# adityaX1412/Experiment-YOLO

Hardware: AMD Instinct MI355X
Metric: images/sec (train) DEAL-YOLO-N 640x640 bs=64/GPU (higher is better)
Workload: dtype f16; 1 GPU; DEAL-YOLO-N (yolov8n-ASF-P2P2.yaml) train step 640x640, per-GPU batch 64, fwd+TAL/WIOU+NWD/DFL/BCE loss+bwd+SGD+EMA, BASELINE.json configs[1]; loss_mode=wiou+nwd, settle_steps=18, capture_retries=0, global_batch=64, parallelism=dp1, hipgraph=True

## Files before the change

### experiment-yolo_amd/csrc/common.h

```cpp
#pragma once
#include <type_traits>
#include <hip/hip_runtime.h>
#include <stdint.h>

typedef _Float16 f16;
typedef _Float16 half8 __attribute__((ext_vector_type(8)));
typedef _Float16 half4 __attribute__((ext_vector_type(4)));
typedef _Float16 half2_ __attribute__((ext_vector_type(2)));
typedef float f32x4 __attribute__((ext_vector_type(4)));
typedef float f32x2 __attribute__((ext_vector_type(2)));

#define DY_OK 0
#define DY_ERR_ARG (-1)
#define DY_ERR_LAUNCH (-2)
#define DY_ERR_ALIGN (-3)
#define DY_ERR_CAPACITY (-4)

#define LDS_AS __attribute__((address_space(3)))

static __device__ __forceinline__ float wave_sum(float v) {
#pragma unroll
  for (int o = 32; o > 0; o >>= 1) v += __shfl_xor(v, o, 64);
  return v;
}
static __device__ __forceinline__ float wave_max(float v) {
#pragma unroll
  for (int o = 32; o > 0; o >>= 1) v = fmaxf(v, __shfl_xor(v, o, 64));
  return v;
}
template <int CTRL>
static __device__ __forceinline__ float dpp_read(float x) {
  return __builtin_bit_cast(float, __builtin_amdgcn_update_dpp(0, __builtin_bit_cast(int, x), CTRL, 0xF, 0xF, true));
}
#define DY_DPP_QUAD_1032 0xB1
#define DY_DPP_QUAD_2301 0x4E
#define DY_DPP_HALF_MIRROR 0x141
// ... 62 lines not shown
    const f32x2 den = (f32x2){__builtin_amdgcn_exp2f(t[0]), __builtin_amdgcn_exp2f(t[1])} + (f32x2){1.f, 1.f};
    const f32x2 s = {__builtin_amdgcn_rcpf(den[0]), __builtin_amdgcn_rcpf(den[1])};
    const f32x2 q = __builtin_elementwise_fma(-s, s, s);
    return __builtin_elementwise_fma(z, q, s);
  }
  if (ACT == DY_ACT_LEAKY) return (f32x2){z[0] > 0.f ? 1.f : 0.1f, z[1] > 0.f ? 1.f : 0.1f};
  return (f32x2){1.f, 1.f};
}
template <int ACT>
static __device__ __forceinline__ float act_grad_t(float z) {
  return act_grad2<ACT>((f32x2){z, z})[0];
}
template <int ACT>
static __device__ __forceinline__ half8 bn_bwd_apply8(const half8& dv, const half8& xv, const float* sc, const float* sh,
                                                      const float* kb, const float* kc) {
  half8 out;
#pragma unroll
  for (int j = 0; j < 8; j += 2) {
    const f32x2 x = {(float)xv[j], (float)xv[j + 1]}, d = {(float)dv[j], (float)dv[j + 1]};
    const f32x2 s2 = {sc[j], sc[j + 1]}, h2 = {sh[j], sh[j + 1]}, b2 = {kb[j], kb[j + 1]}, c2 = {kc[j], kc[j + 1]};
    const f32x2 ad = act_grad2<ACT>(__builtin_elementwise_fma(x, s2, h2));
    const f32x2 o = __builtin_elementwise_fma(s2 * ad, d, -__builtin_elementwise_fma(b2, x, c2));
    const half2_ oh = __builtin_convertvector(o, half2_);
    out[j] = oh[0];
    out[j + 1] = oh[1];
  }
  return out;
}

#define DY_NUM_CUS 256

static inline int cdiv(int a, int b) { return (a + b - 1) / b; }

#define DY_CHECK_LAUNCH()                                  \
  do {                                                     \
    hipError_t e__ = hipGetLastError();                    \
    if (e__ != hipSuccess) return DY_ERR_LAUNCH;           \
  } while (0)
```

### experiment-yolo_amd/csrc/head_rows.hip

```cpp
#include <hip/hip_runtime.h>

#include <cstdlib>

#include "common.h"
#include "dealyolo_hip.h"

template <typename T>
struct Levels {
  int nl;
  T lv[4];
};
struct RowsArgs {
  const f16* x;
  const f16* dy;
  const int* flag;
  const float* w;
  f16* dx;
  float* slabs;
  double* bias_acc;
  int ldx, lddy, lddx, A, a0, hw, B, dx_acc;
  const float* xcoef;
  int nblk, dgx;
};

__global__ __launch_bounds__(256) void rows_wgrad_kernel(Levels<RowsArgs> L) {
  const RowsArgs& a = L.lv[blockIdx.y];
  if ((int)blockIdx.x >= a.nblk) return;
  __shared__ int s_list[256];
  __shared__ int s_cnt[4];
  __shared__ __attribute__((aligned(16))) f16 s_x[16 * 64], s_dy[16 * 64];
  const int tid = threadIdx.x, wave = tid >> 6, lane = tid & 63;
  const int co = tid >> 2, ci0 = (tid & 3) * 16;
  const long npix = (long)a.B * a.hw;
  const long chunk = (npix + a.nblk - 1) / a.nblk;
  const long lo = (long)blockIdx.x * chunk, hi = lo + chunk < npix ? lo + chunk : npix;
  float acc[16];
#pragma unroll
  for (int k = 0; k < 16; ++k) acc[k] = 0.f;
  float bs = 0.f;
  constexpr int FB = 8;
  int fl[FB];
  for (long p0 = lo, trip = 0; p0 < hi; p0 += 256, ++trip) {
    if ((trip & (FB - 1)) == 0) {
#pragma unroll
      for (int k = 0; k < FB; ++k) {
        const long pk = p0 + (long)k * 256 + tid;
        fl[k] = -1;
        if (pk < hi) {
          const int b = (int)(pk / a.hw), r = (int)(pk - (long)b * a.hw);
          fl[k] = a.flag[(size_t)b * a.A + a.a0 + r];
        }
      }
    }
    int mine = -1;
#pragma unroll
    for (int k = 0; k < FB; ++k)
      if ((trip & (FB - 1)) == k) mine = fl[k];
    const bool fg = mine >= 0;
    const unsigned long long m = __ballot(fg);
    if (lane == 0) s_cnt[wave] = __popcll(m);
    __syncthreads();
    int base = 0, total = 0;
#pragma unroll
    for (int w = 0; w < 4; ++w) {
      if (w < wave) base += s_cnt[w];
      total += s_cnt[w];
    }
    if (fg) s_list[base + __popcll(m & ((1ull << lane) - 1ull))] = tid;
    __syncthreads();
    for (int i0 = 0; i0 < total; i0 += 16) {
      const int nb = total - i0 < 16 ? total - i0 : 16;
      {
        const int i = tid >> 4, g = tid & 15;
        if (i < nb) {
          const long q = p0 + s_list[i0 + i];
          if (g < 8) {
            half8 xv = *reinterpret_cast<const half8*>(a.x + q * a.ldx + g * 8);
            if (a.xcoef) xv = bn_silu_apply8(xv, a.xcoef + g * 8, a.xcoef + 64 + g * 8);
            *reinterpret_cast<half8*>(s_x + i * 64 + g * 8) = xv;
          } else {
            *reinterpret_cast<uint4*>(s_dy + i * 64 + (g - 8) * 8) = *reinterpret_cast<const uint4*>(a.dy + q * a.lddy + (g - 8) * 8);
          }
        }
      }
      __syncthreads();
      for (int i = 0; i < nb; ++i) {
        const float g = (float)s_dy[i * 64 + co];
#pragma unroll
        for (int k = 0; k < 16; ++k) acc[k] += g * (float)s_x[i * 64 + ci0 + k];
        if ((tid & 3) == 0) bs += g;
      }
      __syncthreads();
    }
  }
  float* slab = a.slabs + (size_t)blockIdx.x * 64 * 64 + co * 64 + ci0;
#pragma unroll
  for (int k = 0; k < 16; k += 4) *reinterpret_cast<float4*>(slab + k) = make_float4(acc[k], acc[k + 1], acc[k + 2], acc[k + 3]);
  if ((tid & 3) == 0 && bs != 0.f) unsafeAtomicAdd(a.bias_acc + (size_t)(blockIdx.x % DY_BN_COPIES) * 64 + co, (double)bs);
}

__global__ __launch_bounds__(256) void rows_dgrad_kernel(Levels<RowsArgs> L) {
  const RowsArgs& a = L.lv[blockIdx.z];
  if (!a.dx || (int)blockIdx.x >= a.dgx || (int)blockIdx.y >= a.B) return;
  __shared__ float s_w[64 * 65];
  for (int i = threadIdx.x; i < 64 * 64; i += 256) s_w[(i >> 6) * 65 + (i & 63)] = (float)(f16)a.w[i];
  __syncthreads();
  const int b = blockIdx.y, part = threadIdx.x & 7, ci0 = part * 8;
  const int* const fl = a.flag + (size_t)b * a.A + a.a0;
  for (int r = (int)(blockIdx.x * 32 + (threadIdx.x >> 3)); r < a.hw; r += a.dgx * 32) {
    const long p = (long)b * a.hw + r;
    f16* const dst = a.dx + p * a.lddx + ci0;
    if (fl[r] < 0) {
      if (!a.dx_acc) *reinterpret_cast<uint4*>(dst) = make_uint4(0, 0, 0, 0);
      continue;
    }
    float s[8];
#pragma unroll
    for (int k = 0; k < 8; ++k) s[k] = 0.f;
    const f16* const g = a.dy + p * a.lddy;
    for (int c8 = 0; c8 < 64; c8 += 8) {
      const half8 gv = *reinterpret_cast<const half8*>(g + c8);
#pragma unroll
      for (int j = 0; j < 8; ++j) {
        const float gg = (float)gv[j];
#pragma unroll
        for (int k = 0; k < 8; ++k) s[k] += gg * s_w[(c8 + j) * 65 + ci0 + k];
      }
    }
    half8 o;
    if (a.dx_acc) {
      const half8 old = *reinterpret_cast<const half8*>(dst);
#pragma unroll
      for (int k = 0; k < 8; ++k) o[k] = (f16)((float)old[k] + s[k]);
    } else {
#pragma unroll
      for (int k = 0; k < 8; ++k) o[k] = (f16)s[k];
    }
    *reinterpret_cast<half8*>(dst) = o;
  }
}

static __device__ __forceinline__ float exp_nonpos(float x) {
  const float t = x * 1.44269502f;
  float r = __builtin_fmaf(x, 1.44269502f, -t);
  r = __builtin_fmaf(x, 1.92596299e-8f, r);
  const float e = __builtin_amdgcn_exp2f(t);
  return __builtin_fmaf(e, r * 0.693147182f, e);
}
static __device__ __forceinline__ f32x2 exp_nonpos2(f32x2 x) {
  const f32x2 l2e = {1.44269502f, 1.44269502f}, l2e_lo = {1.92596299e-8f, 1.92596299e-8f}, ln2 = {0.693147182f, 0.693147182f};
  const f32x2 t = x * l2e;
  f32x2 r = __builtin_elementwise_fma(x, l2e, -t);
  r = __builtin_elementwise_fma(x, l2e_lo, r);
  const f32x2 e = {__builtin_amdgcn_exp2f(t[0]), __builtin_amdgcn_exp2f(t[1])};
  return __builtin_elementwise_fma(e, r * ln2, e);
}
struct BoxDecArgs {
  const f16* x;
  const float* w;
  const float* bias;
  float* pred_box;
  int ldx, A, a0, hw, W, B;
  const float* xcoef;
  int nblk;
};
template <bool LIBM>
__global__ __launch_bounds__(256) void head_box_decode_kernel(Levels<BoxDecArgs> L) {
  const BoxDecArgs& a = L.lv[blockIdx.y];
  if ((int)blockIdx.x >= a.nblk) return;
  auto ex = [](float x) { return LIBM ? expf(x) : exp_nonpos(x); };
  constexpr int PITCH = 160;
// ... 120 lines not shown
    const int rc = box_decode_fill(L.lv[l], x[l], ldx[l], x_coef ? x_coef[l] : nullptr, weight[l], bias[l], pred_box, A, a0[l], n, h[l], w[l], cin, cout);
    if (rc != DY_OK) return rc;
  }
  return box_decode_launch(L, stream);
}

extern "C" int dy_conv1x1_rows_supported(int cin, int cout) { return cin == 64 && cout == 64; }
extern "C" int dy_conv1x1_rows_slabs(int n, int h, int w) {
  const long ns = (long)n * h * w / 2048;
  return ns < 64 ? 64 : (ns > 1024 ? 1024 : (int)ns);
}
static int rows_fill(RowsArgs& a, const void* x, int ldx, const float* x_coef, const void* dy, int lddy, const int* assigned, int A, int a0,
                     const float* weight, void* dx, int lddx, int dx_accumulate, float* slabs, double* bias_acc, int n, int h, int w, int cin,
                     int cout) {
  if (!dy_conv1x1_rows_supported(cin, cout) || !x || !dy || !assigned || !weight || !slabs || !bias_acc || n < 1 || h < 1 || w < 1 ||
      a0 < 0 || a0 + h * w > A)
    return DY_ERR_ARG;
  if ((ldx & 7) || (lddy & 7) || (dx && (lddx & 7)) || ((uintptr_t)x & 15) || ((uintptr_t)dy & 15) || ((uintptr_t)dx & 15) ||
      ((uintptr_t)slabs & 15))
    return DY_ERR_ALIGN;
  int gx = (h * w + 1023) / 1024;
  if (gx > 16) gx = 16;
  a = RowsArgs{(const f16*)x, (const f16*)dy, assigned, weight, (f16*)dx, slabs, bias_acc, ldx, lddy, lddx, A, a0, h * w, n, dx_accumulate, x_coef,
               dy_conv1x1_rows_slabs(n, h, w), gx};
  return DY_OK;
}
static int rows_launch(const Levels<RowsArgs>& L, hipStream_t stream) {
  int gw = 1, gd = 0, nb = 1;
  for (int l = 0; l < L.nl; ++l) {
    gw = L.lv[l].nblk > gw ? L.lv[l].nblk : gw;
    if (L.lv[l].dx) gd = L.lv[l].dgx > gd ? L.lv[l].dgx : gd;
    nb = L.lv[l].B > nb ? L.lv[l].B : nb;
  }
  hipLaunchKernelGGL(rows_wgrad_kernel, dim3(gw, L.nl), dim3(256), 0, stream, L);
  if (gd) hipLaunchKernelGGL(rows_dgrad_kernel, dim3(gd, nb, L.nl), dim3(256), 0, stream, L);
  DY_CHECK_LAUNCH();
  return DY_OK;
}
extern "C" int dy_conv1x1_rows_backward(const void* x, int ldx, const float* x_coef, const void* dy, int lddy, const int* assigned, int A, int a0,
                                        const float* weight, void* dx, int lddx, int dx_accumulate, float* slabs, double* bias_acc,
                                        int n, int h, int w, int cin, int cout, hipStream_t stream) {
  Levels<RowsArgs> L{};
  L.nl = 1;
  const int rc = rows_fill(L.lv[0], x, ldx, x_coef, dy, lddy, assigned, A, a0, weight, dx, lddx, dx_accumulate, slabs, bias_acc, n, h, w, cin, cout);
  return rc != DY_OK ? rc : rows_launch(L, stream);
}
extern "C" int dy_conv1x1_rows_backward_levels(int nl, const void* const* x, const int* ldx, const float* const* x_coef, const void* const* dy,
                                               const int* lddy, const int* assigned, int A, const int* a0, const float* const* weight,
                                               void* const* dx, const int* lddx, const int* dx_accumulate, float* const* slabs,
                                               double* const* bias_acc, int n, const int* h, const int* w, int cin, int cout,
                                               hipStream_t stream) {
  if (nl < 1 || nl > 4) return DY_ERR_ARG;
  Levels<RowsArgs> L{};
  L.nl = nl;
  for (int l = 0; l < nl; ++l) {
    const int rc = rows_fill(L.lv[l], x[l], ldx[l], x_coef ? x_coef[l] : nullptr, dy[l], lddy[l], assigned, A, a0[l], weight[l], dx[l], lddx[l],
                             dx_accumulate[l], slabs[l], bias_acc[l], n, h[l], w[l], cin, cout);
    if (rc != DY_OK) return rc;
  }
  return rows_launch(L, stream);
}

struct ClsArgs {
  const f16* x;
  const float* xcoef;
  const float* w;
  const float* bias;
  float* y;
// ... 213 lines not shown
```

### experiment-yolo_amd/csrc/loss.hip

```cpp
#include "common.h"
#include "dealyolo_hip.h"

#define REG_MAX 16
#define TOPK 10
#define TAL_EPS 1e-9f
#define IOU_EPS 1e-7f

struct Level {
  const float* box;
  const float* cls;
  f16* dbox;
  f16* dcls;
  int H, W, a0;
  float stride;
  const f16* xin = nullptr;
  int ldin = 0;
  const float* w = nullptr;
  const float* bias = nullptr;
  const float* incoef = nullptr;
};
struct BoxMode {
  int family, ltype, fm, modifier;
  float inner_ratio, focaler_d, focaler_u, shape_scale, piou_lambda;
  float mpd_hw_num;
// ... 317 lines not shown
      const Dual scw = sx * 0.5f + IOU_EPS, sch = sy * 0.5f + IOU_EPS;
      const Dual sigma = t_sqrt(dsq(scw) + dsq(sch));
      const Dual s1 = dabs(scw) / sigma, s2 = dabs(sch) / sigma;
      const Dual sa = dsel(s1.v > 0.70710678118654752f, s2, s1);
      const Dual gamma = dcos(dasin(sa) * 2.f - (float)(M_PI / 2)) - 2.f;
      const Dual dc = (2.f - t_exp(gamma * dsq(scw / cw))) - t_exp(gamma * dsq(sch / ch));
      const Dual ow = dabs(w1 - w2) / dmaximum(w1, dconst(w2)), oh = dabs(h1 - h2) / dmaximum(h1, dconst(h2));
      const Dual sc = dpow4(1.f - t_exp(-ow)) + dpow4(1.f - t_exp(-oh));
      return (I - 0.5f * (dc + sc)) + IOU_EPS;
    }
    case DY_BOX_SHAPEIOU: {
      const float pws = powf(w2, m.shape_scale), phs = powf(h2, m.shape_scale);
      const float ww = 2.f * pws / (pws + phs), hh = 2.f * phs / (pws + phs);
      const Dual dist = (hh * (dsq(sx) / 4.f) + ww * (dsq(sy) / 4.f)) / c2;
      const Dual ow = (hh * dabs(w1 - w2)) / dmaximum(w1, dconst(w2)), oh = (ww * dabs(h1 - h2)) / dmaximum(h1, dconst(h2));
      const Dual sc = dpow4(1.f - t_exp(-ow)) + dpow4(1.f - t_exp(-oh));
      return (I - dist) - 0.5f * sc;
    }
    case DY_BOX_PIOU:
    case DY_BOX_PIOU2: {
      const Dual dw1 = dabs(dminimum(x2, x1) - fminf(t[2], t[0])), dw2 = dabs(dmaximum(x2, x1) - fmaxf(t[2], t[0]));
      const Dual dh1 = dabs(dminimum(y2, y1) - fminf(t[3], t[1])), dh2 = dabs(dmaximum(y2, y1) - fmaxf(t[3], t[1]));
      const Dual P = ((dw1 + dw2) / fabsf(w2) + (dh1 + dh2) / fabsf(h2)) / 4.f;
      const Dual pv1 = ((1.f - I) - t_exp(-dsq(P))) + 1.f;
      if (m.ltype == DY_BOX_PIOU) return 1.f - pv1;
      const Dual x = t_exp(-P) * m.piou_lambda;
      return 1.f - ((3.f * x) * t_exp(-dsq(x))) * pv1;
    }
    default:
      return I - rho2 / c2;
  }
}

__global__ void pack_targets_kernel(LossCtx c, const float* bidx, const float* cls, const float* boxes, int n,
                                    const int* n_dev, float img_w, float img_h) {
  if (n_dev) n = *n_dev;
  for (int i = blockIdx.x * blockDim.x + threadIdx.x; i < c.B * c.nmax; i += gridDim.x * blockDim.x) {
    c.gt_valid[i] = 0;
    c.gt_cls[i] = 0;
    c.pos_align[i] = 0u;
    c.pos_ov[i] = 0u;
    for (int k = 0; k < 4; ++k) c.gt_box[i * 4 + k] = 0.f;
  }
  if (threadIdx.x == 0) c.scal[9] = 0.f;
  __shared__ short sb[8192];
  const int ncache = n < 8192 ? n : 8192;
  for (int i = threadIdx.x; i < ncache; i += blockDim.x) sb[i] = (short)(int)bidx[i];
  __syncthreads();
  for (int i = threadIdx.x; i < n; i += blockDim.x) {
    const int b = (int)bidx[i];
    if (b < 0 || b >= c.B) continue;
    int slot = 0;
    for (int j = 0; j < i; ++j) slot += ((j < ncache ? (int)sb[j] : (int)bidx[j]) == b);
    if (slot >= c.nmax) {
      c.scal[9] = 1.f;
      c.scal[10] = 1.f;
      continue;
    }
    const float x = boxes[i * 4 + 0] * img_w, y = boxes[i * 4 + 1] * img_h;
    const float w = boxes[i * 4 + 2] * img_w, h = boxes[i * 4 + 3] * img_h;
    const float dw = w / 2, dh = h / 2;
    float* g = c.gt_box + ((size_t)b * c.nmax + slot) * 4;
    g[0] = x - dw; g[1] = y - dh; g[2] = x + dw; g[3] = y + dh;
    c.gt_cls[b * c.nmax + slot] = (int)cls[i];
    c.gt_valid[b * c.nmax + slot] = (g[0] + g[1] + g[2] + g[3]) > 0.f ? 1 : 0;
  }
}

static __device__ __forceinline__ float softmax16_expect(float logit, int bin, float& prob) {
  float m = logit;
  m = fmaxf(m, __shfl_xor(m, 1, 64));
  m = fmaxf(m, __shfl_xor(m, 2, 64));
  m = fmaxf(m, __shfl_xor(m, 4, 64));
  m = fmaxf(m, __shfl_xor(m, 8, 64));
  const float e = expf(logit - m);
  const float s = quad16_sum(e);
  prob = e / s;
  return quad16_sum(prob * (float)bin);
}

__global__ __launch_bounds__(256) void decode_kernel(LossCtx c) {
  const int sub = threadIdx.x & 15, side = sub >> 2, quarter = sub & 3;
  const int b = blockIdx.y;
  float invw[4];
#pragma unroll
  for (int k = 0; k < 4; ++k) invw[k] = k < c.nl ? 1.0f / (float)c.lv[k].W : 0.f;
  for (int a = (int)((blockIdx.x * 256 + threadIdx.x) >> 4); a < c.A; a += (int)((gridDim.x * 256) >> 4)) {
    int l = 0;
#pragma unroll
    for (int k = 1; k < 4; ++k)
      if (k < c.nl && a >= c.lv[k].a0) l = k;
    const Level& L = c.lv[l];
    const int r = a - L.a0;
    const int iy = (int)(((float)r + 0.5f) * invw[l]), ix = r - iy * L.W;
    const float4 v = *reinterpret_cast<const float4*>(L.box + ((size_t)b * (L.H * L.W) + r) * 64 + sub * 4);
    float m = fmaxf(fmaxf(v.x, v.y), fmaxf(v.z, v.w));
    m = fmaxf(m, __shfl_xor(m, 1, 64));
    m = fmaxf(m, __shfl_xor(m, 2, 64));
    const float e0 = expf(v.x - m), e1 = expf(v.y - m), e2 = expf(v.z - m), e3 = expf(v.w - m);
    float den = (e0 + e1) + (e2 + e3);
    const float k0 = (float)(quarter * 4);
    float num = e0 * k0 + e1 * (k0 + 1.f) + e2 * (k0 + 2.f) + e3 * (k0 + 3.f);
    den += __shfl_xor(den, 1, 64);
    num += __shfl_xor(num, 1, 64);
    den += __shfl_xor(den, 2, 64);
    num += __shfl_xor(num, 2, 64);
    const float e = num / den;
    const float anc = (side & 1) ? (iy + 0.5f) : (ix + 0.5f);
    if (quarter == 0) c.pred_box[((size_t)b * c.A + a) * 4 + side] = side < 2 ? anc - e : anc + e;
  }
}

#define TAL_CAP 2048
__global__ __launch_bounds__(256) void tal_topk_kernel(LossCtx c) {
  const int bj = blockIdx.x, b = bj / c.nmax, tid = threadIdx.x;
  __shared__ float s_m[TAL_CAP + TOPK];
  __shared__ int s_a[TAL_CAP + TOPK];
  __shared__ float r_m[256];
  __shared__ int r_i[256];
  __shared__ int s_keep;
  int* out = c.topk_idx + (size_t)bj * TOPK;
  if (tid < TOPK) out[tid] = -1;
  if (!c.gt_valid[bj]) return;
  const float* g = c.gt_box + (size_t)bj * 4;
  const float gx1 = g[0], gy1 = g[1], gx2 = g[2], gy2 = g[3];
  const int label = c.gt_cls[bj];
  int x0[4], y0[4], nx[4], ny[4], cum[5];
  cum[0] = 0;
  for (int l = 0; l < 4; ++l) {
    x0[l] = y0[l] = nx[l] = ny[l] = 0;
    if (l < c.nl) {
      const float s = c.lv[l].stride;
      int xa = (int)floorf(gx1 / s - 0.5f) - 1, xb = (int)ceilf(gx2 / s - 0.5f) + 1;
      int ya = (int)floorf(gy1 / s - 0.5f) - 1, yb = (int)ceilf(gy2 / s - 0.5f) + 1;
      xa = xa < 0 ? 0 : xa; ya = ya < 0 ? 0 : ya;
      xb = xb > c.lv[l].W - 1 ? c.lv[l].W - 1 : xb;
      yb = yb > c.lv[l].H - 1 ? c.lv[l].H - 1 : yb;
      x0[l] = xa; y0[l] = ya;
      nx[l] = xb >= xa ? xb - xa + 1 : 0;
      ny[l] = yb >= ya ? yb - ya + 1 : 0;
    }
    cum[l + 1] = cum[l] + nx[l] * ny[l];
  }
  const int ncand = cum[4];
  if (tid == 0) s_keep = 0;
  __syncthreads();
// ... 8 lines not shown
        if (k >= cum[q]) l = q;
      const int r = k - cum[l];
      const int iy = y0[l] + r / nx[l], ix = x0[l] + r % nx[l];
      const float s = c.lv[l].stride;
      const float ax = (ix + 0.5f) * s, ay = (iy + 0.5f) * s;
      const float dmin_ = fminf(fminf(ax - gx1, ay - gy1), fminf(gx2 - ax, gy2 - ay));
      float metric = 0.f;
      const int a = c.lv[l].a0 + iy * c.lv[l].W + ix;
      if (dmin_ > TAL_EPS) {
        const float* pb = c.pred_box + ((size_t)b * c.A + a) * 4;
        const float pp[4] = {pb[0] * s, pb[1] * s, pb[2] * s, pb[3] * s};
        float ov = ciou_gt_pred(g, pp);
        ov = ov > 0.f ? ov : 0.f;
        const float logit = c.lv[l].cls[(((size_t)b * c.lv[l].H + iy) * c.lv[l].W + ix) * c.ncp + label];
        const float sc = c.prob_scores ? logit : 1.f / (1.f + expf(-logit));
        const float o3 = ov * ov * ov;
        metric = sqrtf(sc) * (o3 * o3);
      }
      s_m[keep + t] = metric;
      s_a[keep + t] = a;
    }
    __syncthreads();
    const int n = keep + chunk;
    for (int round = 0; round < TOPK; ++round) {
      float bm = 0.f;
      int bi = -1;
      for (int t = round + tid; t < n; t += 256) {
        const float m = s_m[t];
        if (m > bm || (m == bm && m > 0.f && bi >= 0 && s_a[t] < s_a[bi])) {
          bm = m;
          bi = t;
        }
      }
      r_m[tid] = bm;
      r_i[tid] = bi;
      __syncthreads();
      for (int o = 128; o > 0; o >>= 1) {
        if (tid < o) {
          const float m2 = r_m[tid + o];
          const int i2 = r_i[tid + o];
          const float m1 = r_m[tid];
          const int i1 = r_i[tid];
          if (i2 >= 0 && (i1 < 0 || m2 > m1 || (m2 == m1 && s_a[i2] < s_a[i1]))) {
            r_m[tid] = m2;
            r_i[tid] = i2;
          }
        }
        __syncthreads();
      }
      const int win = r_i[0];
      if (win < 0) {
        if (tid == 0) s_keep = round;
        __syncthreads();
        break;
      }
      if (tid == 0) {
        const float tm = s_m[round];
        const int ta = s_a[round];
        s_m[round] = s_m[win];
        s_a[round] = s_a[win];
        s_m[win] = tm;
        s_a[win] = ta;
        s_keep = round + 1;
      }
      __syncthreads();
    }
    __syncthreads();
  }
  const int keep = s_keep;
  if (tid < keep) out[tid] = s_a[tid];
}

__global__ void tal_scatter_kernel(LossCtx c) {
  const int total = c.B * c.nmax * TOPK;
  for (int i = blockIdx.x * blockDim.x + threadIdx.x; i < total; i += gridDim.x * blockDim.x) {
    const int a = c.topk_idx[i];
    if (a < 0) continue;
    const int bj = i / TOPK, b = bj / c.nmax, j = bj - b * c.nmax;
    atomicAdd(&c.cnt[(size_t)b * c.A + a], 1);
    c.owner[(size_t)b * c.A + a] = j;
  }
}

// ... 85 lines not shown
  __syncthreads();
  for (int o = 128; o > 0; o >>= 1) {
    if (threadIdx.x < o)
      for (int k = 0; k < 3; ++k) red[k][threadIdx.x] += red[k][threadIdx.x + o];
    __syncthreads();
  }
  if (threadIdx.x < 3) c.partials[blockIdx.x * 3 + threadIdx.x] = red[threadIdx.x][0];
}

__global__ __launch_bounds__(256) void loss_scalars_kernel(LossCtx c, int nparts) {
  __shared__ double red[3][256];
  double s[3] = {0, 0, 0};
  for (int i = threadIdx.x; i < nparts; i += 256)
    for (int k = 0; k < 3; ++k) s[k] += c.partials[i * 3 + k];
  for (int k = 0; k < 3; ++k) red[k][threadIdx.x] = s[k];
  __syncthreads();
  for (int o = 128; o > 0; o >>= 1) {
    if (threadIdx.x < o)
      for (int k = 0; k < 3; ++k) red[k][threadIdx.x] += red[k][threadIdx.x + o];
    __syncthreads();
  }
  if (threadIdx.x == 0) {
    const float tss = (float)red[0][0];
    c.scal[0] = tss;
    c.scal[1] = tss > 1.f ? tss : 1.f;
    c.scal[2] = (float)red[1][0];
    c.scal[3] = (float)red[2][0];
    if (c.use_wiou && red[2][0] > 0.0)
      c.scal[4] = c.scal[4] * (1.f - 1e-2f) + 1e-2f * (float)(red[1][0] / red[2][0]);
    c.scal[5] = c.scal[6] = c.scal[7] = c.scal[8] = 0.f;
  }
}

__global__ __launch_bounds__(256) void cls_loss_kernel(LossCtx c, int level) {
  const Level& L = c.lv[level];
  const int hw = L.H * L.W;
  const int npix = c.B * hw;
  const float k = c.hyp_cls * (float)c.B / c.scal[1] * c.gscale[0];
  float acc = 0.f;
  for (int pix = blockIdx.x * 256 + threadIdx.x; pix < npix; pix += gridDim.x * 256) {
    const int b = pix / hw;
    const long ba = (long)b * c.A + L.a0 + (pix - b * hw);
    const int j = c.asg_gt[ba];
    const int tc = j >= 0 ? c.gt_cls[b * c.nmax + j] : -1;
    const float ts = j >= 0 ? c.tscore[ba] : 0.f;
    const float* xp = L.cls + (size_t)pix * c.ncp;
    for (int c0 = 0; c0 < c.ncp; c0 += 8) {
      const float4 v0 = *reinterpret_cast<const float4*>(xp + c0), v1 = *reinterpret_cast<const float4*>(xp + c0 + 4);
      const float xs[8] = {v0.x, v0.y, v0.z, v0.w, v1.x, v1.y, v1.z, v1.w};
      half8 g8;
#pragma unroll
      for (int q = 0; q < 8; ++q) {
        const int cc = c0 + q;
        float g = 0.f;
        if (cc < c.nc) {
          const float x = xs[q], t = cc == tc ? ts : 0.f;
          const float e = __expf(-fabsf(x));
          acc += fmaxf(x, 0.f) - x * t + __logf(1.f + e);
          const float r = __builtin_amdgcn_rcpf(1.f + e);
          g = ((x >= 0.f ? r : e * r) - t) * k;
        }
        g8[q] = (f16)g;
      }
      if (L.dcls) *reinterpret_cast<half8*>(L.dcls + (size_t)pix * c.ncp + c0) = g8;
    }
  }
  __shared__ float red[256];
  red[threadIdx.x] = acc;
  __syncthreads();
  for (int o = 128; o > 0; o >>= 1) {
    if (threadIdx.x < o) red[threadIdx.x] += red[threadIdx.x + o];
    __syncthreads();
  }
  if (threadIdx.x == 0) c.partials[blockIdx.x] = red[0];
}

template <bool EXT>
__global__ __launch_bounds__(256) void box_loss_kernel(LossCtx c) {
  const int lane = threadIdx.x & 63, side = lane >> 4, bin = lane & 15;
  const long wave = ((long)blockIdx.x * 256 + threadIdx.x) >> 6, nw = ((long)gridDim.x * 256) >> 6;
  const long total = (long)c.B * c.A;
  const float tss = c.scal[1], gs = c.gscale[0], Bf = (float)c.B;
  float l_box = 0.f, l_dfl = 0.f;
  for (long base = wave * 64; base < total; base += nw * 64) {
   const int jl = (base + lane < total) ? c.asg_gt[base + lane] : -1;
   unsigned long long fgm = __ballot(jl >= 0);
   while (fgm) {
    const int bit = __ffsll((long long)fgm) - 1;
    fgm &= fgm - 1;
    const long ba = base + bit;
    const int j = __shfl(jl, bit, 64);
    const int b = (int)(ba / c.A), a = (int)(ba - (long)b * c.A);
    int l, iy, ix;
    anchor_of(c, a, l, iy, ix);
    const Level& L = c.lv[l];
    const size_t off = (((size_t)b * L.H + iy) * L.W + ix) * 64 + lane;
    float logit;
    if (L.box) {
      logit = L.box[off];
    } else {
      const float xraw = (float)L.xin[(((size_t)b * L.H + iy) * L.W + ix) * L.ldin + lane];
      float yv = xraw;
      if (L.incoef) {
        const float z = __builtin_fmaf(xraw, L.incoef[lane], L.incoef[64 + lane]);
        const f32x2 a2 = act_fwd2_fast<DY_ACT_SILU>((f32x2){z, z});
        yv = (float)(f16)a2[0];
      }
// ... 157 lines not shown
  return DY_OK;
}

extern "C" int dy_tal_assign(const float* const* scores, const int* H, const int* W, const float* stride, int nl, int B, int nc,
                             int ncp, int n, const float* pd_boxes_grid, const int* gt_labels, const float* gt_bboxes,
                             const int* mask_gt, int* asg_gt, float* tscore, void* workspace, hipStream_t stream) {
  if (nl < 1 || nl > 4 || n < 1 || (ncp & 7) || nc > ncp || !workspace || !asg_gt || !tscore) return DY_ERR_ARG;
  LossCtx c{};
  c.nl = nl; c.B = B; c.nc = nc; c.ncp = ncp; c.nmax = n; c.prob_scores = 1;
  int a0 = 0;
  for (int l = 0; l < nl; ++l) {
    c.lv[l] = Level{nullptr, scores[l], nullptr, nullptr, H[l], W[l], a0, stride[l]};
    a0 += H[l] * W[l];
  }
  c.A = a0;
  char* p = (char*)workspace;
  auto take = [&](size_t b) { char* r = p; p += (b + 255) / 256 * 256; return r; };
  const size_t BA = (size_t)B * c.A, BN = (size_t)B * n;
  take(BN * 16); take(BN * 4); take(BN * 4); take(BA * 16);
  c.gt_box = const_cast<float*>(gt_bboxes); c.gt_cls = const_cast<int*>(gt_labels); c.gt_valid = const_cast<int*>(mask_gt);
  c.pred_box = const_cast<float*>(pd_boxes_grid);
  c.cnt = (int*)take(BA * 4); c.owner = (int*)take(BA * 4);
  take(BA * 4);
  c.asg_gt = asg_gt;
  c.asg_metric = (float*)take(BA * 4); c.asg_ov = (float*)take(BA * 4);
  take(BA * 4);
  c.tscore = tscore;
  c.topk_idx = (int*)take(BN * TOPK * 4); c.pos_align = (unsigned*)take(BN * 4); c.pos_ov = (unsigned*)take(BN * 4);
  take(16 * 4);
  c.partials = (float*)take(3 * 4096 * 4);
  if (hipMemsetAsync(c.cnt, 0, BA * 4, stream) != hipSuccess || hipMemsetAsync(c.pos_align, 0, BN * 4, stream) != hipSuccess ||
      hipMemsetAsync(c.pos_ov, 0, BN * 4, stream) != hipSuccess)
    return DY_ERR_LAUNCH;
  hipLaunchKernelGGL(tal_topk_kernel, dim3((int)BN), dim3(256), 0, stream, c);
  hipLaunchKernelGGL(tal_scatter_kernel, dim3(cdiv((int)BN * TOPK, 256)), dim3(256), 0, stream, c);
  const int gridE = (int)((BA + 255) / 256 < 2048 ? (BA + 255) / 256 : 2048);
  hipLaunchKernelGGL(tal_resolve_kernel, dim3(gridE), dim3(256), 0, stream, c);
  hipLaunchKernelGGL(tal_scores_kernel, dim3(gridE), dim3(256), 0, stream, c);
  DY_CHECK_LAUNCH();
  return DY_OK;
}

extern "C" int dy_loss_args_bytes(void) { return (int)sizeof(DyLossArgs); }
extern "C" int dy_detection_loss(const DyLossArgs* d, hipStream_t stream) {
  if (d->nl < 1 || d->nl > 4 || d->nmax < 1 || (d->ncp & 7) || d->nc > d->ncp) return DY_ERR_ARG;
  LossCtx c{};
  c.nl = d->nl; c.B = d->B; c.nc = d->nc; c.ncp = d->ncp; c.nmax = d->nmax;
  int a0 = 0;
  for (int l = 0; l < d->nl; ++l) {
    c.lv[l] = Level{d->box[l], d->cls[l], (f16*)d->dbox[l], (f16*)d->dcls[l], d->H[l], d->W[l], a0, d->stride[l]};
    if (d->box_from_input) {
      if (!d->box_in[l] || !d->box_w[l] || !d->box_b[l] || (d->box_in_ld[l] & 7)) return DY_ERR_ARG;
      c.lv[l].box = nullptr;
      c.lv[l].xin = (const f16*)d->box_in[l]; c.lv[l].ldin = d->box_in_ld[l]; c.lv[l].w = d->box_w[l]; c.lv[l].bias = d->box_b[l];
      c.lv[l].incoef = d->box_in_coef[l];
    }
    a0 += d->H[l] * d->W[l];
  }
  c.A = a0;
  char* p = (char*)d->workspace;
  auto take = [&](size_t b) { char* r = p; p += (b + 255) / 256 * 256; return r; };
  const size_t BA = (size_t)c.B * c.A, BN = (size_t)c.B * c.nmax;
  c.gt_box = (float*)take(BN * 16); c.gt_cls = (int*)take(BN * 4); c.gt_valid = (int*)take(BN * 4);
  c.pred_box = (float*)take(BA * 16); c.cnt = (int*)take(BA * 4); c.owner = (int*)take(BA * 4);
  c.asg_gt = (int*)take(BA * 4); c.asg_metric = (float*)take(BA * 4); c.asg_ov = (float*)take(BA * 4);
  c.tscore = (float*)take(BA * 4);
  c.topk_idx = (int*)take(BN * TOPK * 4); c.pos_align = (unsigned*)take(BN * 4); c.pos_ov = (unsigned*)take(BN * 4);
  float* scal_ws = (float*)take(16 * 4);
  (void)scal_ws;
  c.scal = d->scalars;
  float* partA = (float*)take(3 * 4096 * 4);
  float* partB = (float*)take(2 * 4096 * 4);
  float* partC = (float*)take(4 * 4096 * 4);
  c.hyp_box = d->hyp_box; c.hyp_cls = d->hyp_cls; c.hyp_dfl = d->hyp_dfl;
  c.use_wiou = d->use_wiou; c.use_nwd = d->use_nwd; c.iou_ratio = d->iou_ratio; c.gscale = d->gscale;
  if (d->box_family != DY_BOX_FAMILY_LEGACY) {
    const int fam = d->box_family, lt = d->box_ltype, mod = d->box_modifier;
    if (fam != DY_BOX_FAMILY_WISE && fam != DY_BOX_FAMILY_BBOX) return DY_ERR_ARG;
    if (lt < DY_BOX_IOU || lt > DY_BOX_MPDIOU || (fam == DY_BOX_FAMILY_BBOX && lt == DY_BOX_WIOU)) return DY_ERR_ARG;
    if (mod < DY_BOX_MOD_PLAIN || mod > DY_BOX_MOD_FOCALER) return DY_ERR_ARG;
    if (fam == DY_BOX_FAMILY_WISE && (d->box_fm < DY_BOX_FM_V1 || d->box_fm > DY_BOX_FM_V3)) return DY_ERR_ARG;
    if (mod == DY_BOX_MOD_FOCALER && !(d->focaler_u != d->focaler_d)) return DY_ERR_ARG;
    c.bm = BoxMode{fam, lt, d->box_fm, mod, d->inner_ratio, d->focaler_d, d->focaler_u, d->shape_scale, d->piou_lambda,
                   d->img_h * d->img_h + d->img_w * d->img_w};
    c.use_wiou = fam == DY_BOX_FAMILY_WISE;
  }

  hipLaunchKernelGGL(pack_targets_kernel, dim3(1), dim3(1024), 0, stream, c, d->t_batch_idx, d->t_cls, d->t_boxes,
                     d->n_targets, d->n_targets_dev, d->img_w, d->img_h);
  if (hipMemsetAsync(c.cnt, 0, BA * 4, stream) != hipSuccess) return DY_ERR_LAUNCH;
  const int gridA = (int)((BA * 64 + 255) / 256 < 2048 ? (BA * 64 + 255) / 256 : 2048);
  if (!d->box_from_input) {
    const long nb = ((long)c.A * 16 + 255) / 256;
    hipLaunchKernelGGL(decode_kernel, dim3((int)(nb < 256 ? nb : 256), c.B), dim3(256), 0, stream, c);
  }
  hipLaunchKernelGGL(tal_topk_kernel, dim3((int)BN), dim3(256), 0, stream, c);
  hipLaunchKernelGGL(tal_scatter_kernel, dim3(cdiv((int)BN * TOPK, 256)), dim3(256), 0, stream, c);
  const int gridE = (int)((BA + 255) / 256 < 2048 ? (BA + 255) / 256 : 2048);
  hipLaunchKernelGGL(tal_resolve_kernel, dim3(gridE), dim3(256), 0, stream, c);
  c.partials = partA;
  hipLaunchKernelGGL(tal_scores_kernel, dim3(gridE), dim3(256), 0, stream, c);
  hipLaunchKernelGGL(loss_scalars_kernel, dim3(1), dim3(256), 0, stream, c, gridE);
  int n_cls = 0;
  for (int l = 0; l < c.nl; ++l) {
    const long tot = (long)c.B * c.lv[l].H * c.lv[l].W;
    int g = (int)((tot + 255) / 256 < 2048 ? (tot + 255) / 256 : 2048);
    c.partials = partC + n_cls;
    hipLaunchKernelGGL(cls_loss_kernel, dim3(g), dim3(256), 0, stream, c, l);
    n_cls += g;
  }
  c.partials = partB;
  for (int l = 0; l < c.nl; ++l)
    if (c.lv[l].dbox && !d->dbox_rows_only && hipMemsetAsync(c.lv[l].dbox, 0, (size_t)c.B * c.lv[l].H * c.lv[l].W * 64 * 2, stream) != hipSuccess)
      return DY_ERR_LAUNCH;
  if (c.bm.family != DY_BOX_FAMILY_LEGACY)
    hipLaunchKernelGGL(box_loss_kernel<true>, dim3(gridA), dim3(256), 0, stream, c);
  else
    hipLaunchKernelGGL(box_loss_kernel<false>, dim3(gridA), dim3(256), 0, stream, c);
  hipLaunchKernelGGL(loss_final_kernel, dim3(1), dim3(256), 0, stream, c, partB, gridA, partC, n_cls);
  DY_CHECK_LAUNCH();
  return DY_OK;
}
```

Measured before the change: 6240 images/s.

## Fuse head row kernels, merge per-level cls loss, speed up target packing and topk

Merges the rows wgrad and dgrad kernels into one launch that splits the grid between the two bodies, and merges the per-level cls_loss launches into a single kernel indexed by level start offsets. Replaces the serial O(n^2) slot counting in target packing with a ballot-based ranking using a shared per-image counter, and replaces the block-wide shared-memory argmax tree in TAL top-k with a wave shuffle reduction plus a 4-entry cross-wave step. The aim is fewer kernel launches and less serialization in small loss kernels. The old paths stay available through the DY_HEAD_V1 environment variable. The new pack kernel zero-fills buffers itself, and the loss path that uses it does not memset pos_align or pos_ov first.

Measured after the change: 6263 images/s (median of 6 runs). No clear change (+0.4%).

```diff
diff --git a/experiment-yolo_amd/csrc/common.h b/experiment-yolo_amd/csrc/common.h
--- a/experiment-yolo_amd/csrc/common.h
+++ b/experiment-yolo_amd/csrc/common.h
@@ -2,6 +2,7 @@
 #include <type_traits>
 #include <hip/hip_runtime.h>
 #include <stdint.h>
+#include <stdlib.h>
 
 typedef _Float16 f16;
 typedef _Float16 half8 __attribute__((ext_vector_type(8)));
@@ -130,6 +131,11 @@
 
 static inline int cdiv(int a, int b) { return (a + b - 1) / b; }
 
+static inline bool dy_head_v1() {
+  const char* e = getenv("DY_HEAD_V1");
+  return e && e[0] == '1' && !e[1];
+}
+
 #define DY_CHECK_LAUNCH()                                  \
   do {                                                     \
     hipError_t e__ = hipGetLastError();                    \
diff --git a/experiment-yolo_amd/csrc/head_rows.hip b/experiment-yolo_amd/csrc/head_rows.hip
--- a/experiment-yolo_amd/csrc/head_rows.hip
+++ b/experiment-yolo_amd/csrc/head_rows.hip
@@ -23,17 +23,18 @@
   int nblk, dgx;
 };
 
-__global__ __launch_bounds__(256) void rows_wgrad_kernel(Levels<RowsArgs> L) {
-  const RowsArgs& a = L.lv[blockIdx.y];
-  if ((int)blockIdx.x >= a.nblk) return;
-  __shared__ int s_list[256];
-  __shared__ int s_cnt[4];
-  __shared__ __attribute__((aligned(16))) f16 s_x[16 * 64], s_dy[16 * 64];
+constexpr int ROWS_LDS = 64 * 65 * 4;
+static __device__ __forceinline__ void rows_wgrad_body(const RowsArgs& a, const int bx, char* smem) {
+  if (bx >= a.nblk) return;
+  int* const s_list = reinterpret_cast<int*>(smem);
+  int* const s_cnt = s_list + 256;
+  f16* const s_x = reinterpret_cast<f16*>(smem + 1040);
+  f16* const s_dy = s_x + 16 * 64;
   const int tid = threadIdx.x, wave = tid >> 6, lane = tid & 63;
   const int co = tid >> 2, ci0 = (tid & 3) * 16;
   const long npix = (long)a.B * a.hw;
   const long chunk = (npix + a.nblk - 1) / a.nblk;
-  const long lo = (long)blockIdx.x * chunk, hi = lo + chunk < npix ? lo + chunk : npix;
+  const long lo = (long)bx * chunk, hi = lo + chunk < npix ? lo + chunk : npix;
   float acc[16];
 #pragma unroll
   for (int k = 0; k < 16; ++k) acc[k] = 0.f;
@@ -93,21 +94,24 @@
       __syncthreads();
     }
   }
-  float* slab = a.slabs + (size_t)blockIdx.x * 64 * 64 + co * 64 + ci0;
+  float* slab = a.slabs + (size_t)bx * 64 * 64 + co * 64 + ci0;
 #pragma unroll
   for (int k = 0; k < 16; k += 4) *reinterpret_cast<float4*>(slab + k) = make_float4(acc[k], acc[k + 1], acc[k + 2], acc[k + 3]);
-  if ((tid & 3) == 0 && bs != 0.f) unsafeAtomicAdd(a.bias_acc + (size_t)(blockIdx.x % DY_BN_COPIES) * 64 + co, (double)bs);
-}
-
-__global__ __launch_bounds__(256) void rows_dgrad_kernel(Levels<RowsArgs> L) {
-  const RowsArgs& a = L.lv[blockIdx.z];
-  if (!a.dx || (int)blockIdx.x >= a.dgx || (int)blockIdx.y >= a.B) return;
-  __shared__ float s_w[64 * 65];
+  if ((tid & 3) == 0 && bs != 0.f) unsafeAtomicAdd(a.bias_acc + (size_t)(bx % DY_BN_COPIES) * 64 + co, (double)bs);
+}
+__global__ __launch_bounds__(256) void rows_wgrad_kernel(Levels<RowsArgs> L) {
+  __shared__ __attribute__((aligned(16))) char smem[1040 + 2 * 16 * 64 * 2];
+  rows_wgrad_body(L.lv[blockIdx.y], (int)blockIdx.x, smem);
+}
+
+static __device__ __forceinline__ void rows_dgrad_body(const RowsArgs& a, const int bx, const int b, char* smem) {
+  if (!a.dx || bx >= a.dgx || b >= a.B) return;
+  float* const s_w = reinterpret_cast<float*>(smem);
   for (int i = threadIdx.x; i < 64 * 64; i += 256) s_w[(i >> 6) * 65 + (i & 63)] = (float)(f16)a.w[i];
   __syncthreads();
-  const int b = blockIdx.y, part = threadIdx.x & 7, ci0 = part * 8;
+  const int part = threadIdx.x & 7, ci0 = part * 8;
   const int* const fl = a.flag + (size_t)b * a.A + a.a0;
-  for (int r = (int)(blockIdx.x * 32 + (threadIdx.x >> 3)); r < a.hw; r += a.dgx * 32) {
+  for (int r = (int)(bx * 32 + (threadIdx.x >> 3)); r < a.hw; r += a.dgx * 32) {
     const long p = (long)b * a.hw + r;
     f16* const dst = a.dx + p * a.lddx + ci0;
     if (fl[r] < 0) {
@@ -137,6 +141,21 @@
       for (int k = 0; k < 8; ++k) o[k] = (f16)s[k];
     }
     *reinterpret_cast<half8*>(dst) = o;
+  }
+}
+__global__ __launch_bounds__(256, 3) void rows_dgrad_kernel(Levels<RowsArgs> L) {
+  __shared__ __attribute__((aligned(16))) char smem[ROWS_LDS];
+  rows_dgrad_body(L.lv[blockIdx.z], (int)blockIdx.x, (int)blockIdx.y, smem);
+}
+__global__ __launch_bounds__(256, 3) void rows_bwd_kernel(Levels<RowsArgs> L, const int gw, const int gd) {
+  __shared__ __attribute__((aligned(16))) char smem[ROWS_LDS];
+  const RowsArgs& a = L.lv[blockIdx.y];
+  const int bx = (int)blockIdx.x;
+  if (bx < gw) {
+    rows_wgrad_body(a, bx, smem);
+  } else {
+    const int i = bx - gw;
+    rows_dgrad_body(a, i % gd, i / gd, smem);
   }
 }
 
@@ -323,8 +342,12 @@
     if (L.lv[l].dx) gd = L.lv[l].dgx > gd ? L.lv[l].dgx : gd;
     nb = L.lv[l].B > nb ? L.lv[l].B : nb;
   }
-  hipLaunchKernelGGL(rows_wgrad_kernel, dim3(gw, L.nl), dim3(256), 0, stream, L);
-  if (gd) hipLaunchKernelGGL(rows_dgrad_kernel, dim3(gd, nb, L.nl), dim3(256), 0, stream, L);
+  if (gd && !dy_head_v1()) {
+    hipLaunchKernelGGL(rows_bwd_kernel, dim3(gw + gd * nb, L.nl), dim3(256), 0, stream, L, gw, gd);
+  } else {
+    hipLaunchKernelGGL(rows_wgrad_kernel, dim3(gw, L.nl), dim3(256), 0, stream, L);
+    if (gd) hipLaunchKernelGGL(rows_dgrad_kernel, dim3(gd, nb, L.nl), dim3(256), 0, stream, L);
+  }
   DY_CHECK_LAUNCH();
   return DY_OK;
 }
diff --git a/experiment-yolo_amd/csrc/loss.hip b/experiment-yolo_amd/csrc/loss.hip
--- a/experiment-yolo_amd/csrc/loss.hip
+++ b/experiment-yolo_amd/csrc/loss.hip
@@ -373,6 +373,21 @@
   }
 }
 
+static __device__ __forceinline__ void pack_fill(const LossCtx& c, const int i, const int b, const int slot, const float* cls,
+                                                 const float* boxes, const float img_w, const float img_h) {
+  if (slot >= c.nmax) {
+    c.scal[9] = 1.f;
+    c.scal[10] = 1.f;
+    return;
+  }
+  const float x = boxes[i * 4 + 0] * img_w, y = boxes[i * 4 + 1] * img_h;
+  const float w = boxes[i * 4 + 2] * img_w, h = boxes[i * 4 + 3] * img_h;
+  const float dw = w / 2, dh = h / 2;
+  float* g = c.gt_box + ((size_t)b * c.nmax + slot) * 4;
+  g[0] = x - dw; g[1] = y - dh; g[2] = x + dw; g[3] = y + dh;
+  c.gt_cls[b * c.nmax + slot] = (int)cls[i];
+  c.gt_valid[b * c.nmax + slot] = (g[0] + g[1] + g[2] + g[3]) > 0.f ? 1 : 0;
+}
 __global__ void pack_targets_kernel(LossCtx c, const float* bidx, const float* cls, const float* boxes, int n,
                                     const int* n_dev, float img_w, float img_h) {
   if (n_dev) n = *n_dev;
@@ -393,18 +408,55 @@
     if (b < 0 || b >= c.B) continue;
     int slot = 0;
     for (int j = 0; j < i; ++j) slot += ((j < ncache ? (int)sb[j] : (int)bidx[j]) == b);
-    if (slot >= c.nmax) {
-      c.scal[9] = 1.f;
-      c.scal[10] = 1.f;
-      continue;
-    }
-    const float x = boxes[i * 4 + 0] * img_w, y = boxes[i * 4 + 1] * img_h;
-    const float w = boxes[i * 4 + 2] * img_w, h = boxes[i * 4 + 3] * img_h;
-    const float dw = w / 2, dh = h / 2;
-    float* g = c.gt_box + ((size_t)b * c.nmax + slot) * 4;
-    g[0] = x - dw; g[1] = y - dh; g[2] = x + dw; g[3] = y + dh;
-    c.gt_cls[b * c.nmax + slot] = (int)cls[i];
-    c.gt_valid[b * c.nmax + slot] = (g[0] + g[1] + g[2] + g[3]) > 0.f ? 1 : 0;
+    pack_fill(c, i, b, slot, cls, boxes, img_w, img_h);
+  }
+}
+
+#define PACK_MAXB 4096
+__global__ __launch_bounds__(1024) void pack_targets_fast_kernel(LossCtx c, const float* bidx, const float* cls, const float* boxes, int n,
+                                                                 const int* n_dev, float img_w, float img_h) {
+  if (n_dev) n = *n_dev;
+  const int tid = threadIdx.x, wave = tid >> 6, lane = tid & 63;
+  for (int i = tid; i < c.B * c.nmax; i += 1024) {
+    c.gt_valid[i] = 0;
+    c.gt_cls[i] = 0;
+    c.pos_align[i] = 0u;
+    c.pos_ov[i] = 0u;
+    for (int k = 0; k < 4; ++k) c.gt_box[i * 4 + k] = 0.f;
+  }
+  if (tid == 0) c.scal[9] = 0.f;
+  __shared__ int s_cnt[PACK_MAXB];
+  for (int i = tid; i < c.B; i += 1024) s_cnt[i] = 0;
+  __syncthreads();
+  for (int base = 0; base < n; base += 1024) {
+    const int i = base + tid;
+    int b = -1;
+    if (i < n) {
+      b = (int)bidx[i];
+      if (b < 0 || b >= c.B) b = -1;
+    }
+    int rank = 0, cnt = 0;
+    unsigned long long todo = __ballot(b >= 0);
+    while (todo) {
+      const int bl = __shfl(b, __ffsll((long long)todo) - 1, 64);
+      const unsigned long long m = __ballot(b == bl);
+      if (b == bl) {
+        rank = __popcll(m & ((1ull << lane) - 1ull));
+        cnt = __popcll(m);
+      }
+      todo &= ~m;
+    }
+    int slot = 0;
+    const int nw = (n - base + 63) / 64 < 16 ? (n - base + 63) / 64 : 16;
+    for (int w = 0; w < nw; ++w) {
+      if (wave == w && b >= 0) {
+        const int before = s_cnt[b];
+        slot = before + rank;
+        if (rank == cnt - 1) s_cnt[b] = before + cnt;
+      }
+      __syncthreads();
+    }
+    if (b >= 0) pack_fill(c, i, b, slot, cls, boxes, img_w, img_h);
   }
 }
 
@@ -453,6 +505,7 @@
 }
 
 #define TAL_CAP 2048
+template <bool TREE>
 __global__ __launch_bounds__(256) void tal_topk_kernel(LossCtx c) {
   const int bj = blockIdx.x, b = bj / c.nmax, tid = threadIdx.x;
   __shared__ float s_m[TAL_CAP + TOPK];
@@ -527,6 +580,39 @@
           bi = t;
         }
       }
+      int win;
+      if constexpr (!TREE) {
+        int ba = bi >= 0 ? s_a[bi] : 0;
+#pragma unroll
+        for (int o = 32; o > 0; o >>= 1) {
+          const float m2 = __shfl_xor(bm, o, 64);
+          const int a2 = __shfl_xor(ba, o, 64), i2 = __shfl_xor(bi, o, 64);
+          if (i2 >= 0 && (bi < 0 || m2 > bm || (m2 == bm && a2 < ba))) {
+            bm = m2;
+            ba = a2;
+            bi = i2;
+          }
+        }
+        if ((tid & 63) == 0) {
+          r_m[tid >> 6] = bm;
+          r_i[tid >> 6] = bi;
+          r_i[4 + (tid >> 6)] = ba;
+        }
+        __syncthreads();
+        float wm = r_m[0];
+        int wi = r_i[0], wa = r_i[4];
+#pragma unroll
+        for (int w = 1; w < 4; ++w) {
+          const float m2 = r_m[w];
+          const int i2 = r_i[w], a2 = r_i[4 + w];
+          if (i2 >= 0 && (wi < 0 || m2 > wm || (m2 == wm && a2 < wa))) {
+            wm = m2;
+            wa = a2;
+            wi = i2;
+          }
+        }
+        win = wi;
+      } else {
       r_m[tid] = bm;
       r_i[tid] = bi;
       __syncthreads();
@@ -543,7 +629,8 @@
         }
         __syncthreads();
       }
-      const int win = r_i[0];
+      win = r_i[0];
+      }
       if (win < 0) {
         if (tid == 0) s_keep = round;
         __syncthreads();
@@ -695,13 +782,13 @@
   }
 }
 
-__global__ __launch_bounds__(256) void cls_loss_kernel(LossCtx c, int level) {
+static __device__ __forceinline__ void cls_loss_body(const LossCtx& c, const int level, const int bx, const int gx, float* part) {
   const Level& L = c.lv[level];
   const int hw = L.H * L.W;
   const int npix = c.B * hw;
   const float k = c.hyp_cls * (float)c.B / c.scal[1] * c.gscale[0];
   float acc = 0.f;
-  for (int pix = blockIdx.x * 256 + threadIdx.x; pix < npix; pix += gridDim.x * 256) {
+  for (int pix = bx * 256 + threadIdx.x; pix < npix; pix += gx * 256) {
     const int b = pix / hw;
     const long ba = (long)b * c.A + L.a0 + (pix - b * hw);
     const int j = c.asg_gt[ba];
@@ -735,7 +822,21 @@
     if (threadIdx.x < o) red[threadIdx.x] += red[threadIdx.x + o];
     __syncthreads();
   }
-  if (threadIdx.x == 0) c.partials[blockIdx.x] = red[0];
+  if (threadIdx.x == 0) *part = red[0];
+}
+__global__ __launch_bounds__(256) void cls_loss_kernel(LossCtx c, int level) {
+  cls_loss_body(c, level, (int)blockIdx.x, (int)gridDim.x, c.partials + blockIdx.x);
+}
+struct ClsLossGrid {
+  int start[5];
+};
+__global__ __launch_bounds__(256) void cls_loss_levels_kernel(LossCtx c, ClsLossGrid g) {
+  const int bx = (int)blockIdx.x;
+  int l = 0;
+#pragma unroll
+  for (int k = 1; k < 4; ++k)
+    if (k < c.nl && bx >= g.start[k]) l = k;
+  cls_loss_body(c, l, bx - g.start[l], g.start[l + 1] - g.start[l], c.partials + bx);
 }
 
 template <bool EXT>
@@ -959,7 +1060,8 @@
   if (hipMemsetAsync(c.cnt, 0, BA * 4, stream) != hipSuccess || hipMemsetAsync(c.pos_align, 0, BN * 4, stream) != hipSuccess ||
       hipMemsetAsync(c.pos_ov, 0, BN * 4, stream) != hipSuccess)
     return DY_ERR_LAUNCH;
-  hipLaunchKernelGGL(tal_topk_kernel, dim3((int)BN), dim3(256), 0, stream, c);
+  if (dy_head_v1()) hipLaunchKernelGGL(tal_topk_kernel<true>, dim3((int)BN), dim3(256), 0, stream, c);
+  else hipLaunchKernelGGL(tal_topk_kernel<false>, dim3((int)BN), dim3(256), 0, stream, c);
   hipLaunchKernelGGL(tal_scatter_kernel, dim3(cdiv((int)BN * TOPK, 256)), dim3(256), 0, stream, c);
   const int gridE = (int)((BA + 255) / 256 < 2048 ? (BA + 255) / 256 : 2048);
   hipLaunchKernelGGL(tal_resolve_kernel, dim3(gridE), dim3(256), 0, stream, c);
@@ -1013,15 +1115,21 @@
     c.use_wiou = fam == DY_BOX_FAMILY_WISE;
   }
 
-  hipLaunchKernelGGL(pack_targets_kernel, dim3(1), dim3(1024), 0, stream, c, d->t_batch_idx, d->t_cls, d->t_boxes,
-                     d->n_targets, d->n_targets_dev, d->img_w, d->img_h);
+  const bool v1 = dy_head_v1();
+  if (v1 || c.B > PACK_MAXB)
+    hipLaunchKernelGGL(pack_targets_kernel, dim3(1), dim3(1024), 0, stream, c, d->t_batch_idx, d->t_cls, d->t_boxes,
+                       d->n_targets, d->n_targets_dev, d->img_w, d->img_h);
+  else
+    hipLaunchKernelGGL(pack_targets_fast_kernel, dim3(1), dim3(1024), 0, stream, c, d->t_batch_idx, d->t_cls, d->t_boxes,
+                       d->n_targets, d->n_targets_dev, d->img_w, d->img_h);
   if (hipMemsetAsync(c.cnt, 0, BA * 4, stream) != hipSuccess) return DY_ERR_LAUNCH;
   const int gridA = (int)((BA * 64 + 255) / 256 < 2048 ? (BA * 64 + 255) / 256 : 2048);
   if (!d->box_from_input) {
     const long nb = ((long)c.A * 16 + 255) / 256;
     hipLaunchKernelGGL(decode_kernel, dim3((int)(nb < 256 ? nb : 256), c.B), dim3(256), 0, stream, c);
   }
-  hipLaunchKernelGGL(tal_topk_kernel, dim3((int)BN), dim3(256), 0, stream, c);
+  if (dy_head_v1()) hipLaunchKernelGGL(tal_topk_kernel<true>, dim3((int)BN), dim3(256), 0, stream, c);
+  else hipLaunchKernelGGL(tal_topk_kernel<false>, dim3((int)BN), dim3(256), 0, stream, c);
   hipLaunchKernelGGL(tal_scatter_kernel, dim3(cdiv((int)BN * TOPK, 256)), dim3(256), 0, stream, c);
   const int gridE = (int)((BA + 255) / 256 < 2048 ? (BA + 255) / 256 : 2048);
   hipLaunchKernelGGL(tal_resolve_kernel, dim3(gridE), dim3(256), 0, stream, c);
@@ -1029,12 +1137,18 @@
   hipLaunchKernelGGL(tal_scores_kernel, dim3(gridE), dim3(256), 0, stream, c);
   hipLaunchKernelGGL(loss_scalars_kernel, dim3(1), dim3(256), 0, stream, c, gridE);
   int n_cls = 0;
+  ClsLossGrid cg{};
   for (int l = 0; l < c.nl; ++l) {
     const long tot = (long)c.B * c.lv[l].H * c.lv[l].W;
     int g = (int)((tot + 255) / 256 < 2048 ? (tot + 255) / 256 : 2048);
     c.partials = partC + n_cls;
-    hipLaunchKernelGGL(cls_loss_kernel, dim3(g), dim3(256), 0, stream, c, l);
+    if (v1) hipLaunchKernelGGL(cls_loss_kernel, dim3(g), dim3(256), 0, stream, c, l);
     n_cls += g;
+    cg.start[l + 1] = n_cls;
+  }
+  if (!v1) {
+    c.partials = partC;
+    hipLaunchKernelGGL(cls_loss_levels_kernel, dim3(n_cls), dim3(256), 0, stream, c, cg);
   }
   c.partials = partB;
   for (int l = 0; l < c.nl; ++l)
```
